# MECLabTUDA/Lifelong-nnUNet

Measured on AMD Instinct MI355X. Metric: 3D patches/sec (whole node) + mean Dice vs ref, 5-level 3D Generic_UNet training step, higher is better.
Workload: dtype f16 (fp32 accumulate, fp32 master weights); 1 GPU; BASELINE configs[1]: nnUNetTrainerSequential.run_iteration, 160x192x160 patches, batch 2/GPU, num_pool 5, base 32, 3 logits; global_batch=2, parallelism=dp1, distinct_resident_batches=2, deterministic_wgrad=False

## Files before the change

lifelong-nnunet_amd/csrc/igemm_common.h:

```cpp
#pragma once
#include "lnn_common.h"

struct TapTable {
    int ntaps;
    int taps_per_group;
    unsigned short pos_off[27];
    unsigned char slot[27];
};

struct ConvParams {
    const half_t* x;
    const half_t* x2;
    half_t* y2;
    int csplit = 0x7fffffff, msplit = 0x7fffffff;
    const half_t* wp;
    const float* bias;
    half_t* y;
    int ld_x, ld_y;
    int N, Di, Hi, Wi, Do, Ho, Wo;
    int C, M, Mpad, KCpad;
    int wtaps;
    int Ld, Lh, Lw;
    int tiles_z, tiles_y, tiles_x;
    int os, par_z, par_y, par_x;
// ... 8 lines not shown
    int gs_in[3] = {0, 0, 0}, gs_out[3] = {0, 0, 0};
    long gs_in_n = 0, gs_out_n = 0;
    unsigned gs_nrec_in = 0, gs_nrec_out = 0;
    int ksplit = 1;
    float* scratch = nullptr;
    unsigned long long* dbg;
    TapTable taps;
};


__host__ __device__ __forceinline__ long lnn_panel_off(int slot, int m, int kc, int wtaps, int KCpad) {
    return ((((long)(m >> 5) * (KCpad >> 4) + (kc >> 4)) * wtaps + slot) * 32 + (m & 31)) * 16 + (kc & 15);
}

int lnn_launch_conv_s1_tile(hipStream_t s, ConvParams& p, const char* name);
bool lnn_conv_s1_v9_supported(const ConvParams& p);
int lnn_conv_s1_v9_stats_slots(const ConvParams& p);
bool lnn_conv_s1_v9_red_supported(const ConvParams& p);
int lnn_launch_splitk_finalize(hipStream_t s, const ConvParams& p, const char* name);
int lnn_launch_in_small_fwd(hipStream_t s, const void* y, void* z, int ld_z, int N, long V, int C, float eps, const float* gamma,
                            const float* beta, float slope, float* mean, float* rstd);
int lnn_launch_in_small_bwd(hipStream_t s, void* y, const void* dz, int ld_dz, int N, long V, int C, const float* mean, const float* rstd,
                            const float* gamma, const float* beta, float slope, double* ws, float* dgamma, float* dbeta, float unscale);
int lnn_launch_in_stats_finalize(hipStream_t s, const float* pws, int nslots, int N, int C, long V, float eps, float* mean, float* rstd);
int lnn_launch_in_bwd_sums_raw(hipStream_t s, const float* pws, int nslots, int N, int C, const float* mean, const float* rstd,
                               double* ws, float* dgamma, float* dbeta, float unscale);
int lnn_launch_conv_s1_v9(hipStream_t s, ConvParams& p, const char* name);
int lnn_conv_k133_on_v9(hipStream_t s, const void* x, int ld_x, const void* wp, const float* bias, void* y, int ld_y, int N, int D, int H,
                        int W, int C, int M, int flip, const char* name);
bool lnn_conv_s1_mt_supported(const ConvParams& p);
double lnn_conv_s1_mt_efficiency(const ConvParams& p);
int lnn_conv_s1_mt_ksplit(const ConvParams& p, const float* ws, long ws_elems);
int lnn_launch_conv_s1_mt(hipStream_t s, ConvParams& p, float* ws, long ws_elems, const char* name);
int lnn_launch_up2_dgrad(hipStream_t s, ConvParams& p, const char* name);
int lnn_launch_up2_convT(hipStream_t s, ConvParams& p, const char* name);
int lnn_launch_down2_conv(hipStream_t s, ConvParams& p, const char* name);
int lnn_launch_down2_convT_dgrad(hipStream_t s, ConvParams& p, const char* name);
bool lnn_down2s_supported(const ConvParams& p);
int lnn_down2s_stats_slots(const ConvParams& p);
int lnn_launch_down2s(hipStream_t s, ConvParams& p, const char* name);
```

lifelong-nnunet_amd/csrc/igemm_conv.hip:

```cpp
#include "lnn_common.h"
#include "igemm_common.h"
#include "igemm_gen.h"
#include <cstdlib>

namespace {

typedef unsigned c1_uint4 __attribute__((ext_vector_type(4)));

template <bool STATS>
__global__ __launch_bounds__(256, 3) void conv_c1_fwd_kernel(const ConvParams p, int tiles_per_sample) {
    constexpr int TZ = 4, TY = 8, TX = 8, VT = TZ * TY * TX / 128, PZ = TZ + 2, PY = TY + 2, PX = TX + 2, P = PZ * PY * PX;
    constexpr int NL = (P + 255) / 256;
    __shared__ half_t xl[P];
    __shared__ float sred[STATS ? 4 * 2 * 32 : 1];
    const int tid = threadIdx.x, lane = tid & 63, wave = tid >> 6;
    const int n = blockIdx.y;
    const int m0 = blockIdx.z * 32;
    const long xbase_n = (long)n * p.Di * p.Hi * p.Wi;
    const int v = lane & 31, hk = lane >> 5;
    half8 a[2];
#pragma unroll
    for (int k16 = 0; k16 < 2; ++k16) a[k16] = *reinterpret_cast<const half8*>(p.wp + lnn_panel_off(0, m0 + v, k16 * 16 + hk * 8, 1, 32));
    int toff[2][8];
#pragma unroll
// ... 122 lines not shown
    if (v == 1) return true;
    static int min_planes = 0;
    if (!min_planes) { const char* e = getenv("LNN_CONV_V9_MIN_PLANES"); min_planes = e && atoi(e) > 0 ? atoi(e) : 16; }
    return p.Ld >= min_planes;
}

int g_force_down2 = -1;
bool use_down2s(const ConvParams& p) {
    if (!lnn_down2s_supported(p)) return false;
    if (g_force_down2 >= 0) return g_force_down2 == 1;
    static int v = -2;
    if (v == -2) {
        const char* e = getenv("LNN_DOWN2S");
        v = e ? (e[0] == '1' ? 1 : 0) : -1;
    }
    if (v == 0) return false;
    if (v == 1) return true;
    return p.Ld >= 16;
}

bool use_mt(const ConvParams& p) {
    if (!lnn_conv_s1_mt_supported(p)) return false;
    if (g_force_conv >= 0) return g_force_conv == 10;
    static int v = -2;
    if (v == -2) {
        const char* e = getenv("LNN_CONV_MT");
        v = e ? (e[0] == '1' ? 1 : 0) : -1;
    }
    if (v == 0) return false;
    if (v == 1) return true;
    return p.C >= 128;
}

}

static int g_gen_mode = -1;
extern "C" int lnn_debug_set_gen_mode(int mode) {
    LNN_REQUIRE(mode >= -1 && mode <= 1, "lnn_debug_set_gen_mode: %d is not one of -1, 0, 1", mode);
    g_gen_mode = mode;
    return LNN_OK;
}
bool lnn_gen_prefers(int op, long voxels) {
    if (g_gen_mode >= 0) return g_gen_mode == 1;
    if (g_force_conv >= 0) return false;
    static int off = -1;
    if (off < 0) { const char* e = getenv("LNN_GEN"); off = (e && e[0] == '0') ? 1 : 0; }
    if (off) return false;
    switch (op) {
        case LNN_GEN_OP_CONV_S1: return voxels > 512 && voxels <= 4096;
        case LNN_GEN_OP_CONV_S2: return voxels <= 4096;
        case LNN_GEN_OP_CONVT_DGRAD: return voxels <= 20000;
        default: return false;
    }
}

namespace {
int check_act(const void* ptr, int ld, int C, const char* what) {
    LNN_REQUIRE(ptr != nullptr, "%s: null pointer", what);
    LNN_REQUIRE(lnn_aligned16(ptr), "%s: pointer not 16-byte aligned", what);
    LNN_REQUIRE(C > 0 && C % 8 == 0, "%s: channel count %d must be a positive multiple of 8", what, C);
    LNN_REQUIRE(ld >= C && ld % 8 == 0, "%s: ld %d must be >= C (%d) and a multiple of 8", what, ld, C);
    return LNN_OK;
}

}

extern "C" int lnn_debug_force_down2_kernel(int which) {
    LNN_REQUIRE(which >= -1 && which <= 1, "lnn_debug_force_down2_kernel: %d is not one of -1, 0, 1", which);
    g_force_down2 = which;
    return LNN_OK;
}

extern "C" int lnn_debug_force_conv_kernel(int which) {
    LNN_REQUIRE(which == -1 || which == 5 || which == 9 || which == 10, "lnn_debug_force_conv_kernel: %d is not one of -1, 5, 9, 10", which);
    g_force_conv = which;
    return LNN_OK;
}

namespace {
int conv3d_fwd_impl(lnn_stream_t s_, const void* x, const void* x2, int c_a, int ld_x, const void* wp, const float* bias, void* y,
                    int ld_y, int N, int Di, int Hi, int Wi, int C, int K, int stride, float* stats_pws = nullptr,
                    int* stats_slots = nullptr, float* splitk_ws = nullptr, long splitk_elems = 0) {
    hipStream_t s = (hipStream_t)s_;
    LNN_REQUIRE(stride == 1 || stride == 2, "lnn_conv3d_fwd: stride %d unsupported", stride);
    LNN_REQUIRE(N > 0 && Di > 0 && Hi > 0 && Wi > 0, "lnn_conv3d_fwd: bad dims");
    LNN_REQUIRE(wp != nullptr && lnn_aligned16(wp), "lnn_conv3d_fwd: weight panel null/misaligned");
    LNN_REQUIRE(bias == nullptr || lnn_aligned16(bias), "lnn_conv3d_fwd: bias misaligned");
    if (int e = check_act(y, ld_y, K, "lnn_conv3d_fwd(y)")) return e;
    ConvParams p{};
    p.x = (const half_t*)x; p.wp = (const half_t*)wp; p.bias = bias; p.y = (half_t*)y;
    if (x2) { p.x2 = (const half_t*)x2; p.csplit = c_a; }
    p.ld_x = ld_x; p.ld_y = ld_y; p.N = N; p.Di = Di; p.Hi = Hi; p.Wi = Wi;
    p.Do = (Di - 1) / stride + 1; p.Ho = (Hi - 1) / stride + 1; p.Wo = (Wi - 1) / stride + 1;
    p.C = C; p.M = K; p.Mpad = lnn_round_up(K, 32); p.wtaps = C == 1 ? 1 : 27;
    p.Ld = p.Do; p.Lh = p.Ho; p.Lw = p.Wo; p.os = 1; p.pad_lo = 1; p.accumulate = 0;
    if (C == 1) {
        LNN_REQUIRE(stride == 1, "lnn_conv3d_fwd: C == 1 path supports stride 1 only");
        LNN_REQUIRE(x != nullptr, "lnn_conv3d_fwd: null x");
        p.KCpad = 32;
        p.tiles_z = lnn_cdiv(p.Ld, 4); p.tiles_y = lnn_cdiv(p.Lh, 8); p.tiles_x = lnn_cdiv(p.Lw, 8);
        const int tps = p.tiles_z * p.tiles_y * p.tiles_x;
        int nb = 768 / N;
        if (nb < 1) nb = 1;
        if (nb > tps) nb = tps;
        dim3 grid((unsigned)nb, (unsigned)N, (unsigned)lnn_cdiv(K, 32));
        if (stats_pws && ld_y == K) {
            p.stats_pws = stats_pws;
            p.stats_nblk = nb;
            hipLaunchKernelGGL((conv_c1_fwd_kernel<true>), grid, dim3(256), 0, s, p, tps);
            *stats_slots = nb;
        } else {
            hipLaunchKernelGGL((conv_c1_fwd_kernel<false>), grid, dim3(256), 0, s, p, tps);
        }
        LNN_CHECK_LAUNCH("lnn_conv3d_fwd(C=1)");
        return LNN_OK;
    }
    if (int e = check_act(x, ld_x, x2 ? c_a : C, "lnn_conv3d_fwd(x)")) return e;
    p.KCpad = lnn_round_up(C, 16);
    p.taps.ntaps = 27;
    if (stride == 1) {
        constexpr int PY = 10, PX = 10;
        for (int t = 0; t < 27; ++t) {
            p.taps.pos_off[t] = (unsigned short)(((t / 9) * PY + (t / 3) % 3) * PX + t % 3);
            p.taps.slot[t] = (unsigned char)t;
        }
        if (!use_v9(p) && use_mt(p)) return lnn_launch_conv_s1_mt(s, p, splitk_ws, splitk_elems, "lnn_conv3d_fwd(s1,mt)");
    }
    if (!x2 && lnn_gen_prefers(stride == 1 ? LNN_GEN_OP_CONV_S1 : LNN_GEN_OP_CONV_S2, (long)N * p.Do * p.Ho * p.Wo)) {
        const int k3[3] = {3, 3, 3}, st3[3] = {stride, stride, stride};
        return lnn_gen_conv3d_fwd(s, x, ld_x, wp, bias, y, ld_y, N, Di, Hi, Wi, C, K, k3, st3, splitk_ws, splitk_elems);
    }
    if (stride == 1) {
        p.dbg = g_dbg;
        if (stats_pws && use_v9(p) && ld_y == K && lnn_conv_s1_v9_stats_slots(p) <= 1024) {
            p.stats_pws = stats_pws;
            const int rc = lnn_launch_conv_s1_v9(s, p, "lnn_conv3d_fwd(s1,v9,stats)");
            *stats_slots = p.stats_nblk;
            return rc;
        }
        if (use_v9(p)) return lnn_launch_conv_s1_v9(s, p, "lnn_conv3d_fwd(s1,v9)");
        return lnn_launch_conv_s1_tile(s, p, "lnn_conv3d_fwd(s1,v5)");
    }
    if (use_down2s(p)) {
        if (stats_pws && ld_y == K && lnn_down2s_stats_slots(p) <= 1024) {
            p.stats_pws = stats_pws;
            const int rc = lnn_launch_down2s(s, p, "lnn_conv3d_fwd(s2,down2s,stats)");
            *stats_slots = p.stats_nblk;
            return rc;
        }
        return lnn_launch_down2s(s, p, "lnn_conv3d_fwd(s2,down2s)");
    }
    return lnn_launch_down2_conv(s, p, "lnn_conv3d_fwd(s2,down2)");
}

int check_cat(const void* b, int c_a, int C, int stride, const char* what) {
    LNN_REQUIRE(b != nullptr && lnn_aligned16(b), "%s: second tensor null/misaligned", what);
    LNN_REQUIRE(stride == 1, "%s: stride 1 only", what);
    LNN_REQUIRE(c_a > 0 && c_a < C && c_a % 32 == 0 && (C - c_a) % 8 == 0, "%s: split %d of %d channels must be a multiple of 32", what, c_a, C);
    return LNN_OK;
}
// ... 178 lines not shown
    hipStream_t s = (hipStream_t)s_;
    LNN_REQUIRE(wp != nullptr && lnn_aligned16(wp), "lnn_convT3d_k2s2_fwd: weight panel null/misaligned");
    if (int e = check_act(x, ld_x, C, "lnn_convT3d_k2s2_fwd(x)")) return e;
    if (int e = check_act(y, ld_y, K, "lnn_convT3d_k2s2_fwd(y)")) return e;
    if (lnn_gen_prefers(LNN_GEN_OP_CONVT_FWD, (long)N * D * H * W * 8)) {
        const int st3[3] = {2, 2, 2};
        return lnn_gen_convT3d_fwd(s, x, ld_x, wp, y, ld_y, N, D, H, W, C, K, st3, ws, ws_elems);
    }
    ConvParams p{};
    p.x = (const half_t*)x; p.wp = (const half_t*)wp; p.y = (half_t*)y; p.ld_x = ld_x; p.ld_y = ld_y;
    p.N = N; p.Di = D; p.Hi = H; p.Wi = W; p.Do = 2 * D; p.Ho = 2 * H; p.Wo = 2 * W;
    p.C = C; p.M = K; p.Mpad = lnn_round_up(K, 32); p.KCpad = lnn_round_up(C, 16); p.wtaps = 8;
    p.Ld = D; p.Lh = H; p.Lw = W; p.os = 2; p.pad_lo = 0;
    return lnn_launch_up2_convT(s, p, "lnn_convT3d_k2s2_fwd(up2)");
}
}

extern "C" int lnn_convT3d_k2s2_fwd(lnn_stream_t s, const void* x, int ld_x, const void* wp, void* y, int ld_y, int N,
                                    int D, int H, int W, int C, int K) {
    return convT3d_k2s2_fwd_impl(s, x, ld_x, wp, y, ld_y, N, D, H, W, C, K, nullptr, 0);
}
extern "C" int lnn_convT3d_k2s2_fwd_ws(lnn_stream_t s, const void* x, int ld_x, const void* wp, void* y, int ld_y, int N,
                                       int D, int H, int W, int C, int K, float* splitk_ws, long splitk_elems) {
    return convT3d_k2s2_fwd_impl(s, x, ld_x, wp, y, ld_y, N, D, H, W, C, K, splitk_ws, splitk_elems);
}

namespace {
int convT3d_k2s2_dgrad_impl(lnn_stream_t s_, const void* dy, int ld_dy, const void* wp, void* dx, int ld_dx, int N, int D, int H, int W,
                            int C, int K, int accumulate, float* ws, long ws_elems) {
    hipStream_t s = (hipStream_t)s_;
    LNN_REQUIRE(wp != nullptr && lnn_aligned16(wp), "lnn_convT3d_k2s2_dgrad: weight panel null/misaligned");
    if (int e = check_act(dy, ld_dy, K, "lnn_convT3d_k2s2_dgrad(dy)")) return e;
    if (int e = check_act(dx, ld_dx, C, "lnn_convT3d_k2s2_dgrad(dx)")) return e;
    if (lnn_gen_prefers(LNN_GEN_OP_CONVT_DGRAD, (long)N * D * H * W)) {
        const int st3[3] = {2, 2, 2};
        return lnn_gen_convT3d_dgrad(s, dy, ld_dy, wp, dx, ld_dx, N, D, H, W, C, K, st3, accumulate, ws, ws_elems);
    }
    ConvParams p{};
    p.x = (const half_t*)dy; p.wp = (const half_t*)wp; p.y = (half_t*)dx; p.ld_x = ld_dy; p.ld_y = ld_dx;
    p.N = N; p.Di = 2 * D; p.Hi = 2 * H; p.Wi = 2 * W; p.Do = D; p.Ho = H; p.Wo = W;
    p.C = K; p.M = C; p.Mpad = lnn_round_up(C, 32); p.KCpad = lnn_round_up(K, 16); p.wtaps = 8;
    p.Ld = D; p.Lh = H; p.Lw = W; p.os = 1; p.pad_lo = 0; p.accumulate = accumulate;
    if (use_down2s(p)) return lnn_launch_down2s(s, p, "lnn_convT3d_k2s2_dgrad(down2s)");
    return lnn_launch_down2_convT_dgrad(s, p, "lnn_convT3d_k2s2_dgrad(down2)");
}
}

extern "C" int lnn_convT3d_k2s2_dgrad(lnn_stream_t s, const void* dy, int ld_dy, const void* wp, void* dx, int ld_dx,
                                      int N, int D, int H, int W, int C, int K, int accumulate) {
    return convT3d_k2s2_dgrad_impl(s, dy, ld_dy, wp, dx, ld_dx, N, D, H, W, C, K, accumulate, nullptr, 0);
}
extern "C" int lnn_convT3d_k2s2_dgrad_ws(lnn_stream_t s, const void* dy, int ld_dy, const void* wp, void* dx, int ld_dx,
                                         int N, int D, int H, int W, int C, int K, int accumulate, float* splitk_ws, long splitk_elems) {
    return convT3d_k2s2_dgrad_impl(s, dy, ld_dy, wp, dx, ld_dx, N, D, H, W, C, K, accumulate, splitk_ws, splitk_elems);
}
```

lifelong-nnunet_amd/csrc/igemm_conv_mt.hip:

```cpp
#include "igemm_common.h"

namespace {

typedef unsigned uint4v __attribute__((ext_vector_type(4)));
typedef __attribute__((address_space(3))) void lds_void;

template <int N>
__device__ __forceinline__ void mt_wait_vm() {
    static_assert(N == 0 || N == 4 || N == 6 || N == 8 || N == 10 || N == 12, "extend the table");
    if constexpr (N == 0) asm volatile("s_waitcnt vmcnt(0)" ::: "memory");
    if constexpr (N == 4) asm volatile("s_waitcnt vmcnt(4)" ::: "memory");
    if constexpr (N == 6) asm volatile("s_waitcnt vmcnt(6)" ::: "memory");
    if constexpr (N == 8) asm volatile("s_waitcnt vmcnt(8)" ::: "memory");
    if constexpr (N == 10) asm volatile("s_waitcnt vmcnt(10)" ::: "memory");
    if constexpr (N == 12) asm volatile("s_waitcnt vmcnt(12)" ::: "memory");
}

__device__ __forceinline__ void mt_dma16(__amdgpu_buffer_rsrc_t rs, char* lds_wave_base, int voffset, int soffset) {
    __builtin_amdgcn_raw_ptr_buffer_load_lds(rs, (lds_void*)lds_wave_base, 16, voffset, soffset, 0, 0);
}

constexpr int MT_NW = 8;
constexpr int MT_NH = 4;
constexpr int MT_HALO = MT_NW * MT_NH * 1024;
constexpr int mt_lds(int AR) { return 2 * MT_HALO + MT_NW * AR * 2048; }
constexpr int MT_NIT = 7;

struct MTLaunch {
    int mblk;
    int zb, yb, xb;
    int TY, TX, PY, PX, P;
    int cpp;
    int nbands;
};

template <int WN, int MT_AR>
__global__ __launch_bounds__(512, 2) void igemm_conv_mt_kernel(const ConvParams p, const MTLaunch q) {
    static_assert(MT_AR >= 3 && MT_AR <= 7, "ring depth");
    extern __shared__ __attribute__((aligned(16))) char smem[];
    char* const aring = smem + 2 * MT_HALO;
    const int tid = threadIdx.x, lane = tid & 63;
    const int wave = __builtin_amdgcn_readfirstlane(tid >> 6);
    const int sub = wave >> 2, kq = wave & 3;
// ... 234 lines not shown
    }
    return lnn_cu_budget(num_cu);
}

bool mt_geometry(const ConvParams& p, int& WN, int& TY, int& TX, double& eff) {
    WN = 0; TY = 0; TX = 0; eff = 0.0;
    for (int nx = 1; nx <= 16; ++nx) {
        const int tx = lnn_cdiv(p.Lw, nx);
        if (nx > 1 && tx == lnn_cdiv(p.Lw, nx - 1)) continue;
        for (int wn = 5; wn >= 4; --wn) {
            int ty = (32 * wn) / tx;
            if (ty > p.Lh) ty = p.Lh;
            while (ty >= 1 && 4L * (ty + 2) * (tx + 2) > MT_NW * MT_NH * 32) --ty;
            if (ty < 1) continue;
            const double e = (double)p.Lh * p.Lw / ((double)lnn_cdiv(p.Lh, ty) * lnn_cdiv(p.Lw, tx) * 32 * wn);
            if (e > eff + 1e-9) { eff = e; WN = wn; TY = ty; TX = tx; }
        }
    }
    return WN != 0;
}

template <int WN, int AR>
int launch_mt(hipStream_t s, ConvParams& p, const MTLaunch& q, int grid, const char* name) {
    static bool attr_set = false;
    if (!attr_set) {
        (void)hipFuncSetAttribute(reinterpret_cast<const void*>(igemm_conv_mt_kernel<WN, AR>), hipFuncAttributeMaxDynamicSharedMemorySize, mt_lds(AR));
        attr_set = true;
    }
    hipLaunchKernelGGL((igemm_conv_mt_kernel<WN, AR>), dim3(grid), dim3(512), mt_lds(AR), s, p, q);
    LNN_CHECK_LAUNCH(name);
    return LNN_OK;
}

}

int lnn_launch_splitk_finalize(hipStream_t s, const ConvParams& p, const char* name) {
    const long nvox = (long)p.N * p.Do * p.Ho * p.Wo;
    const long total = nvox * (p.Mpad >> 2);
    const int blocks = (int)((total + 255) / 256 < 4096 ? (total + 255) / 256 : 4096);
    hipLaunchKernelGGL(splitk_finalize_kernel, dim3(blocks), dim3(256), 0, s, p, nvox);
    LNN_CHECK_LAUNCH(name);
    return LNN_OK;
}

bool lnn_conv_s1_mt_supported(const ConvParams& p) {
    if (p.os != 1 || p.pad_lo != 1 || p.taps.ntaps != 27 || p.wtaps != 27) return false;
    if (p.C % 16 != 0 || p.Mpad % 32 != 0 || p.M % 8 != 0) return false;
    if (p.ld_x % 8 != 0 || p.ld_y % 8 != 0) return false;
    if (p.csplit != 0x7fffffff && p.csplit % 16 != 0) return false;
    if (p.msplit != 0x7fffffff && p.msplit % 32 != 0) return false;
    if (p.Di != p.Do || p.Hi != p.Ho || p.Wi != p.Wo) return false;
    if ((double)p.Di * p.Hi * p.Wi * p.ld_x * 2.0 >= 2147483648.0) return false;
    if ((double)p.Mpad * p.KCpad * 27 * 2.0 >= 2147483648.0) return false;
    int wn, ty, tx; double eff;
    return mt_geometry(p, wn, ty, tx, eff);
}

double lnn_conv_s1_mt_efficiency(const ConvParams& p) {
    int wn, ty, tx; double eff;
    if (!lnn_conv_s1_mt_supported(p) || !mt_geometry(p, wn, ty, tx, eff)) return 0.0;
    return eff * p.Ld / (2.0 * lnn_cdiv(p.Ld, 2));
}

int lnn_conv_s1_mt_ksplit(const ConvParams& p, const float* ws, long ws_elems) {
    int wn, ty, tx; double eff;
    if (!mt_geometry(p, wn, ty, tx, eff)) return 1;
// ... 30 lines not shown
```

lifelong-nnunet_amd/csrc/lnn_debug.h:

```cpp
#ifndef LNN_DEBUG_H
#define LNN_DEBUG_H
#include "../../include/lnn_hip.h"
#ifdef __cplusplus
extern "C" {
#endif

int lnn_debug_tr16_probe(lnn_stream_t s, float* out256);

int lnn_debug_set_phase_buffer(void* dev_ptr_6x_u64);
int lnn_debug_force_conv_kernel(int which);
int lnn_debug_force_down2_kernel(int which);
int lnn_debug_set_v9_zseg(int segments);

int lnn_debug_set_k133_v9(int mode);
int lnn_debug_last_k133_on_v9(void);

int lnn_debug_set_gen_mode(int mode);

int lnn_debug_last_dgrad_reduce_fused(void);

int lnn_debug_set_cu_budget(int cus);

#ifdef __cplusplus
}
#endif
#endif
```

lifelong-nnunet_amd/engine.py:

```python
from __future__ import annotations

from dataclasses import dataclass, field
from typing import List, Optional

import os

import torch

from . import native as nat

LRELU_SLOPE = 1e-2
IN_EPS = 1e-5


class Act:

    def __init__(self, buf: torch.Tensor, off: int, C: int):
        self.buf, self.off, self.C = buf, off, C
        self.ld = buf.shape[-1]
        self.N = buf.shape[0]
        self.dims = tuple(buf.shape[1:4])
        self.V = self.dims[0] * self.dims[1] * self.dims[2]

    def data_ptr(self):
# ... 340 lines not shown
        self._pack_total, self._unpack_total = pk_total, up_total
        cmax = max(2 * f for f in feats)
        ws_doubles = max(nat.query("lnn_instnorm_ws_doubles", N, cmax), (nat.query("lnn_seg1x1_bwd_ws_floats", N, cmax) + 1) // 2,
                         nat.query("lnn_instnorm_lrelu_seg_bwd_ws_doubles", N, max(seg.cin for seg in self.segs)), 64)
        self.ws = torch.zeros(ws_doubles, dtype=torch.float64, device=dev)
        need = 1
        for blk in self.blocks:
            if blk.stride != 1 or blk.cin_k == 1:
                continue
            od = blk.in_dims
            vox = N * od[0] * od[1] * od[2]
            tiles = N * -(-od[0] // 8) * -(-od[1] // 8) * -(-od[2] // 8)
            for ch in (blk.cout, blk.cin):
                if tiles * -(-ch // 32) < 512:
                    need = max(need, 8 * vox * (-(-ch // 32) * 32))

        def gen_need(vox, ch, classes=1, always=False, limit=4096):
            if vox > limit and not always:
                return 1
            mp = -(-ch // 32) * 32
            waves = classes * -(-(vox // classes) // 64) * -(-mp // 64)
            ks = 1
            while waves * ks * 2 <= 2048 and ks < 64:
                ks *= 2
            return ks * vox * mp if ks > 1 else 1
        for blk in self.blocks:
            if blk.cin_k == 1:
                continue
            ncls = blk.strides[0] * blk.strides[1] * blk.strides[2]
            need = max(need, gen_need(N * blk.z.V, blk.cout, 1, not blk.iso))
            need = max(need, gen_need(N * blk.in_dims[0] * blk.in_dims[1] * blk.in_dims[2], blk.cin_k, ncls, not blk.iso))
        for up in self.ups:
            need = max(need, gen_need(N * up.y.V, up.cout, up.ntaps, not up.iso), gen_need(N * up.x.V, up.cin, 1, not up.iso, 20000))
        self.splitk_ws = torch.zeros(need, dtype=torch.float32, device=dev)
        self.packed_version = -1
        self.unused_heads: List[str] = []
        self._sides = {}
        self.overlap_wgrad = os.environ.get("LNN_NO_WGRAD_OVERLAP", "0") != "1"
        self.deterministic_wgrad = os.environ.get("LNN_DETERMINISTIC_WGRAD", "0") == "1"
        self._det_buf = None
        self.fuse_seg_fwd = os.environ.get("LNN_NO_FUSED_SEG", "0") != "1"
        self.numeric_conv_bias_grad = os.environ.get("LNN_NUMERIC_CONV_BIAS_GRAD", "0") == "1"
        self.fuse_in_stats = os.environ.get("LNN_NO_FUSED_IN_STATS", "0") != "1"
        self.fuse_seg_bwd = os.environ.get("LNN_NO_FUSED_SEG_BWD", "0") != "1"
        self.fuse_first_bwd = os.environ.get("LNN_NO_FUSED_FIRST_BWD", "0") != "1"
        self.fuse_in_bwd_reduce = os.environ.get("LNN_NO_FUSED_IN_BWD_REDUCE", "0") != "1"
        self.small_v = nat.query("lnn_instnorm_small_volume") if os.environ.get("LNN_IN_SMALL", "1") != "0" else 0
        self.probe = None
        self._watermark = {}
        for item in order:
            slots = [s for s in (getattr(item, a, None) for a in ("w", "b", "gamma", "beta")) if s is not None]
            self._watermark[id(item)] = max(s.offset + (s.numel + 3) // 4 * 4 for s in slots)

    def _probed(self, kind, item, fn):
        pr = self.probe
        if pr is None or (pr.get("layer") != item.prefix and pr.get("layer") != "*"):
            fn()
            return
        e0, e1 = torch.cuda.Event(enable_timing=True), torch.cuda.Event(enable_timing=True)
        e0.record()
        fn()
        e1.record()
        if pr.get("layer") == "*":
            pr.setdefault("all", []).append((item.prefix, kind, e0, e1))
        else:
            pr.setdefault(kind, []).append((e0, e1))
# ... 377 lines not shown
```

lifelong-nnunet_amd/native.py:

```python
from __future__ import annotations

import ctypes as C
import os

_HERE = os.path.dirname(os.path.abspath(__file__))
LIB_PATH = os.environ.get("LNN_LIB_PATH") or os.path.join(_HERE, "csrc", "liblnn_hip.so")

_p = C.c_void_p
_i = C.c_int
_l = C.c_long
_f = C.c_float
_sz = C.c_size_t

SIGNATURES = {
    "lnn_last_error": (C.c_char_p, []),
    "lnn_version": (_i, []),
    "lnn_device_info": (_i, [C.POINTER(_i), C.POINTER(_i), C.c_char_p, _i]),
    "lnn_pack_weights": (_i, [_p, _p, _p, _i, _i, _i, _l, _l, _l]),
    "lnn_packed_weight_elems": (_sz, [_i, _i, _i]),
    "lnn_conv3d_fwd": (_i, [_p, _p, _i, _p, _p, _p, _i, _i, _i, _i, _i, _i, _i, _i]),
    "lnn_conv3d_dgrad": (_i, [_p, _p, _i, _p, _p, _i, _i, _i, _i, _i, _i, _i, _i, _i]),
    "lnn_conv3d_wgrad": (_i, [_p, _p, _i, _p, _i, _p, _i, _i, _i, _i, _i, _i, _i]),
    "lnn_conv3d_fwd_cat": (_i, [_p, _p, _p, _i, _i, _p, _p, _p, _i, _i, _i, _i, _i, _i, _i]),
    "lnn_conv3d_fwd_in_stats": (_i, [_p, _p, _p, _i, _i, _p, _p, _p, _i, _i, _i, _i, _i, _i, _i, _f, _p, _p, _p, _p, _l]),
# ... 45 lines not shown
    "lnn_fisher_ema": (_i, [_p, _p, _p, _l, _f, _f]),
    "lnn_rw_update": (_i, [_p, _p, _p, _p, _p, _p, _l, _f, _f, _p, _f, _f, _i]),
    "lnn_target_ce_fwd": (_i, [_p, _p, _p, _i, _i, _i, _l, _f, _i, _f, _p, _p]),
    "lnn_target_ce_bwd": (_i, [_p, _p, _p, _i, _i, _i, _l, _f, _i, _f, _p, _f, _p, _p]),
    "lnn_softmax_accumulate": (_i, [_p, _p, _p, _p, _p] + [_i] * 11 + [_f, _i]),
    "lnn_softmax_finalize": (_i, [_p, _p, _p, _i, _l, _p]),
    "lnn_gradnorm_sumsq": (_i, [_p, _p, _l, _f, _p, _i]),
    "lnn_flat_reduce_ws_doubles": (_sz, []),
    "lnn_sgd_nesterov_step_clipped": (_i, [_p, _p, _p, _p, _l, _f, _f, _f, _f, _f, _p]),
    "lnn_sgd_nesterov_step": (_i, [_p, _p, _p, _p, _l, _f, _f, _f, _f, _i]),
    "lnn_cast_f32_to_h": (_i, [_p, _p, _p, _l]),
    "lnn_f32_conv3d_fwd": (_i, [_p, _p, _i, _p, _p, _p, _i, _i, _i, _i, _i, _i, _i, _i]),
    "lnn_f32_conv3d_dgrad": (_i, [_p, _p, _i, _p, _p, _i, _i, _i, _i, _i, _i, _i, _i, _i]),
    "lnn_f32_conv3d_wgrad": (_i, [_p, _p, _i, _p, _i, _p, _i, _i, _i, _i, _i, _i, _i]),
    "lnn_f32_convT3d_k2s2_fwd": (_i, [_p, _p, _i, _p, _p, _i, _i, _i, _i, _i, _i, _i]),
    "lnn_f32_convT3d_k2s2_dgrad": (_i, [_p, _p, _i, _p, _p, _i, _i, _i, _i, _i, _i, _i, _i]),
    "lnn_f32_convT3d_k2s2_wgrad": (_i, [_p, _p, _i, _p, _i, _p, _i, _i, _i, _i, _i, _i]),
    "lnn_f32_conv3d_fwd_g": (_i, [_p, _p, _i, _p, _p, _p, _i] + [_i] * 12),
    "lnn_f32_conv3d_dgrad_g": (_i, [_p, _p, _i, _p, _p, _i] + [_i] * 13),
    "lnn_f32_conv3d_wgrad_g": (_i, [_p, _p, _i, _p, _i, _p] + [_i] * 12),
    "lnn_f32_convT3d_fwd_g": (_i, [_p, _p, _i, _p, _p, _i] + [_i] * 9),
    "lnn_f32_convT3d_dgrad_g": (_i, [_p, _p, _i, _p, _p, _i] + [_i] * 10),
    "lnn_f32_convT3d_wgrad_g": (_i, [_p, _p, _i, _p, _i, _p] + [_i] * 9),
    "lnn_image_to_cl_h": (_i, [_p, _p, _p, _i, _i, _l, _i]),
    "lnn_f32_image_to_cl": (_i, [_p, _p, _p, _i, _i, _l, _i]),
    "lnn_f32_instnorm_lrelu_fwd": (_i, [_p, _p, _i, _p, _i, _i, _l, _i, _f, _p, _p, _p, _p, _f]),
    "lnn_f32_instnorm_lrelu_bwd": (_i, [_p, _p, _i, _p, _i, _i, _l, _i, _p, _p, _p, _p, _f, _p, _p, _p]),
    "lnn_f32_seg1x1_fwd": (_i, [_p, _p, _i, _p, _p, _i, _l, _i, _i]),
    "lnn_f32_seg1x1_bwd": (_i, [_p, _p, _i, _p, _p, _p, _i, _p, _i, _l, _i, _i, _i]),
    "lnn_debug_tr16_probe": (_i, [_p, _p]),
    "lnn_debug_set_phase_buffer": (_i, [_p]),
    "lnn_debug_force_conv_kernel": (_i, [_i]),
    "lnn_debug_force_down2_kernel": (_i, [_i]),
    "lnn_debug_set_v9_zseg": (_i, [_i]),
    "lnn_debug_set_k133_v9": (_i, [_i]),
    "lnn_debug_last_k133_on_v9": (_i, []),
    "lnn_debug_set_gen_mode": (_i, [_i]),
    "lnn_debug_last_dgrad_reduce_fused": (_i, []),
    "lnn_debug_set_cu_budget": (_i, [_i]),
    "lnn_conv3d_fwd_g": (_i, [_p, _p, _i, _p, _p, _p, _i] + [_i] * 12 + [_p, _l]),
    "lnn_conv3d_dgrad_g": (_i, [_p, _p, _i, _p, _p, _i] + [_i] * 13 + [_p, _l]),
    "lnn_conv3d_wgrad_g": (_i, [_p, _p, _i, _p, _i, _p] + [_i] * 12 + [_p, _l]),
    "lnn_convT3d_fwd_g": (_i, [_p, _p, _i, _p, _p, _i] + [_i] * 9 + [_p, _l]),
    "lnn_convT3d_dgrad_g": (_i, [_p, _p, _i, _p, _p, _i] + [_i] * 10 + [_p, _l]),
    "lnn_convT3d_wgrad_g": (_i, [_p, _p, _i, _p, _i, _p] + [_i] * 9 + [_p, _l]),
    "lnn_convT3d_k2s2_fwd_ws": (_i, [_p, _p, _i, _p, _p, _i, _i, _i, _i, _i, _i, _i, _p, _l]),
    "lnn_convT3d_k2s2_dgrad_ws": (_i, [_p, _p, _i, _p, _p, _i, _i, _i, _i, _i, _i, _i, _i, _p, _l]),
}

_lib = None


class NativeLibraryMissing(RuntimeError):
    pass


def lib():
    global _lib
    if _lib is None:
        if not os.path.exists(LIB_PATH):
            raise NativeLibraryMissing(
                f"{LIB_PATH} not found: build it with `python -c 'import __graft_entry__ as g; g.build()'` "
                f"(make -C lifelong-nnunet_amd/csrc).  There is no CPU / PyTorch fallback.")
        h = C.CDLL(LIB_PATH)
        for name, (res, args) in SIGNATURES.items():
            fn = getattr(h, name)
# ... 56 lines not shown
```

Baseline: 104.3 patches/s.

## Add stride-2 macro-tile implicit-GEMM kernel for downsampling conv and convT dgrad

Adds a new MFMA macro-tile kernel for stride-2 3x3x3 forward convolutions and 2x2x2 transposed-conv data gradients. It stages a phase-split halo band in LDS with double-buffered DMA and a ring of weight fragments, and splits taps across four waves followed by an LDS reduction. Optional split-K uses a scratch workspace, which is sized in the engine. It is chosen for iso layers with C>=128, more than 512 voxels and good tile efficiency, replacing the generic and down2 kernels there. This adds kernel complexity and LDS pressure and could pick a slower path on some shapes.

```diff
diff --git a/lifelong-nnunet_amd/csrc/igemm_common.h b/lifelong-nnunet_amd/csrc/igemm_common.h
--- a/lifelong-nnunet_amd/csrc/igemm_common.h
+++ b/lifelong-nnunet_amd/csrc/igemm_common.h
@@ -64,6 +64,10 @@
 double lnn_conv_s1_mt_efficiency(const ConvParams& p);
 int lnn_conv_s1_mt_ksplit(const ConvParams& p, const float* ws, long ws_elems);
 int lnn_launch_conv_s1_mt(hipStream_t s, ConvParams& p, float* ws, long ws_elems, const char* name);
+bool lnn_conv_s2_mt_supported(const ConvParams& p);
+double lnn_conv_s2_mt_efficiency(const ConvParams& p);
+long lnn_conv_s2_mt_scratch_elems(const ConvParams& p);
+int lnn_launch_conv_s2_mt(hipStream_t s, ConvParams& p, float* ws, long ws_elems, const char* name);
 int lnn_launch_up2_dgrad(hipStream_t s, ConvParams& p, const char* name);
 int lnn_launch_up2_convT(hipStream_t s, ConvParams& p, const char* name);
 int lnn_launch_down2_conv(hipStream_t s, ConvParams& p, const char* name);
diff --git a/lifelong-nnunet_amd/csrc/igemm_conv.hip b/lifelong-nnunet_amd/csrc/igemm_conv.hip
--- a/lifelong-nnunet_amd/csrc/igemm_conv.hip
+++ b/lifelong-nnunet_amd/csrc/igemm_conv.hip
@@ -178,6 +178,23 @@
     return p.C >= 128;
 }
 
+int g_last_s2_kernel = 0;
+int g_gen_mode_pinned();
+bool use_s2mt(const ConvParams& p, bool have_x2) {
+    if (have_x2 || !lnn_conv_s2_mt_supported(p)) return false;
+    if (g_force_down2 >= 0) return g_force_down2 == 2;
+    if (g_gen_mode_pinned() >= 0 || g_force_conv >= 0) return false;
+    static int v = -2;
+    if (v == -2) {
+        const char* e = getenv("LNN_CONV_S2MT");
+        v = e ? (e[0] == '1' ? 1 : 0) : -1;
+    }
+    if (v == 0) return false;
+    if (v == 1) return true;
+    const long vox = (long)p.N * p.Do * p.Ho * p.Wo;
+    return p.wtaps == 27 && p.C >= 128 && vox > 512 && lnn_conv_s2_mt_efficiency(p) >= 0.7;
+}
+
 }
 
 static int g_gen_mode = -1;
@@ -186,6 +203,7 @@
     g_gen_mode = mode;
     return LNN_OK;
 }
+namespace { int g_gen_mode_pinned() { return g_gen_mode; } }
 bool lnn_gen_prefers(int op, long voxels) {
     if (g_gen_mode >= 0) return g_gen_mode == 1;
     if (g_force_conv >= 0) return false;
@@ -212,9 +230,27 @@
 }
 
 extern "C" int lnn_debug_force_down2_kernel(int which) {
-    LNN_REQUIRE(which >= -1 && which <= 1, "lnn_debug_force_down2_kernel: %d is not one of -1, 0, 1", which);
+    LNN_REQUIRE(which >= -1 && which <= 2, "lnn_debug_force_down2_kernel: %d is not one of -1, 0, 1, 2", which);
     g_force_down2 = which;
     return LNN_OK;
+}
+extern "C" int lnn_debug_last_s2_kernel(void) { return g_last_s2_kernel; }
+
+extern "C" long lnn_conv_s2_mt_scratch_elems_q(int ext, int N, int D, int H, int W, int C, int K) {
+    ConvParams p{};
+    p.N = N; p.os = 1; p.ld_x = 8; p.ld_y = 8;
+    if (ext == 3) {
+        p.Di = D; p.Hi = H; p.Wi = W; p.Do = (D - 1) / 2 + 1; p.Ho = (H - 1) / 2 + 1; p.Wo = (W - 1) / 2 + 1;
+        p.C = C; p.M = K; p.wtaps = 27; p.pad_lo = 1; p.ld_x = lnn_round_up(C, 8);
+    } else if (ext == 2) {
+        p.Di = 2 * D; p.Hi = 2 * H; p.Wi = 2 * W; p.Do = D; p.Ho = H; p.Wo = W;
+        p.C = K; p.M = C; p.wtaps = 8; p.pad_lo = 0; p.ld_x = lnn_round_up(K, 8);
+    } else {
+        return 0;
+    }
+    p.Mpad = lnn_round_up(p.M, 32); p.KCpad = lnn_round_up(p.C, 16);
+    p.Ld = p.Do; p.Lh = p.Ho; p.Lw = p.Wo;
+    return lnn_conv_s2_mt_scratch_elems(p);
 }
 
 extern "C" int lnn_debug_force_conv_kernel(int which) {
@@ -272,6 +308,13 @@
         }
         if (!use_v9(p) && use_mt(p)) return lnn_launch_conv_s1_mt(s, p, splitk_ws, splitk_elems, "lnn_conv3d_fwd(s1,mt)");
     }
+    if (stride == 2) {
+        g_last_s2_kernel = 0;
+        if (use_s2mt(p, x2 != nullptr)) {
+            g_last_s2_kernel = 2;
+            return lnn_launch_conv_s2_mt(s, p, splitk_ws, splitk_elems, "lnn_conv3d_fwd(s2,mt)");
+        }
+    }
     if (!x2 && lnn_gen_prefers(stride == 1 ? LNN_GEN_OP_CONV_S1 : LNN_GEN_OP_CONV_S2, (long)N * p.Do * p.Ho * p.Wo)) {
         const int k3[3] = {3, 3, 3}, st3[3] = {stride, stride, stride};
         return lnn_gen_conv3d_fwd(s, x, ld_x, wp, bias, y, ld_y, N, Di, Hi, Wi, C, K, k3, st3, splitk_ws, splitk_elems);
@@ -516,15 +559,20 @@
     LNN_REQUIRE(wp != nullptr && lnn_aligned16(wp), "lnn_convT3d_k2s2_dgrad: weight panel null/misaligned");
     if (int e = check_act(dy, ld_dy, K, "lnn_convT3d_k2s2_dgrad(dy)")) return e;
     if (int e = check_act(dx, ld_dx, C, "lnn_convT3d_k2s2_dgrad(dx)")) return e;
-    if (lnn_gen_prefers(LNN_GEN_OP_CONVT_DGRAD, (long)N * D * H * W)) {
-        const int st3[3] = {2, 2, 2};
-        return lnn_gen_convT3d_dgrad(s, dy, ld_dy, wp, dx, ld_dx, N, D, H, W, C, K, st3, accumulate, ws, ws_elems);
-    }
     ConvParams p{};
     p.x = (const half_t*)dy; p.wp = (const half_t*)wp; p.y = (half_t*)dx; p.ld_x = ld_dy; p.ld_y = ld_dx;
     p.N = N; p.Di = 2 * D; p.Hi = 2 * H; p.Wi = 2 * W; p.Do = D; p.Ho = H; p.Wo = W;
     p.C = K; p.M = C; p.Mpad = lnn_round_up(C, 32); p.KCpad = lnn_round_up(K, 16); p.wtaps = 8;
     p.Ld = D; p.Lh = H; p.Lw = W; p.os = 1; p.pad_lo = 0; p.accumulate = accumulate;
+    g_last_s2_kernel = 0;
+    if (use_s2mt(p, false)) {
+        g_last_s2_kernel = 2;
+        return lnn_launch_conv_s2_mt(s, p, ws, ws_elems, "lnn_convT3d_k2s2_dgrad(s2,mt)");
+    }
+    if (lnn_gen_prefers(LNN_GEN_OP_CONVT_DGRAD, (long)N * D * H * W)) {
+        const int st3[3] = {2, 2, 2};
+        return lnn_gen_convT3d_dgrad(s, dy, ld_dy, wp, dx, ld_dx, N, D, H, W, C, K, st3, accumulate, ws, ws_elems);
+    }
     if (use_down2s(p)) return lnn_launch_down2s(s, p, "lnn_convT3d_k2s2_dgrad(down2s)");
     return lnn_launch_down2_convT_dgrad(s, p, "lnn_convT3d_k2s2_dgrad(down2)");
 }
diff --git a/lifelong-nnunet_amd/csrc/igemm_conv_mt.hip b/lifelong-nnunet_amd/csrc/igemm_conv_mt.hip
--- a/lifelong-nnunet_amd/csrc/igemm_conv_mt.hip
+++ b/lifelong-nnunet_amd/csrc/igemm_conv_mt.hip
@@ -7,8 +7,9 @@
 
 template <int N>
 __device__ __forceinline__ void mt_wait_vm() {
-    static_assert(N == 0 || N == 4 || N == 6 || N == 8 || N == 10 || N == 12, "extend the table");
+    static_assert(N == 0 || N == 2 || N == 4 || N == 6 || N == 8 || N == 10 || N == 12, "extend the table");
     if constexpr (N == 0) asm volatile("s_waitcnt vmcnt(0)" ::: "memory");
+    if constexpr (N == 2) asm volatile("s_waitcnt vmcnt(2)" ::: "memory");
     if constexpr (N == 4) asm volatile("s_waitcnt vmcnt(4)" ::: "memory");
     if constexpr (N == 6) asm volatile("s_waitcnt vmcnt(6)" ::: "memory");
     if constexpr (N == 8) asm volatile("s_waitcnt vmcnt(8)" ::: "memory");
@@ -309,6 +310,330 @@
     return LNN_OK;
 }
 
+constexpr int S2_NH = 6;
+constexpr int S2_HALO = MT_NW * S2_NH * 1024;
+constexpr int S2_AR = 4;
+constexpr int S2_LDS = 2 * S2_HALO + MT_NW * S2_AR * 2048;
+static_assert(S2_LDS <= 160 * 1024, "the stride-2 macro-tile kernel needs more LDS than a CU has");
+constexpr int S2_SUBP_MAX = MT_NW * S2_NH * 32 / 2;
+
+struct S2Launch {
+    int mblk, zb, yb, xb;
+    int TY, TX, PY, PX, SUBP;
+    int cpp, nbands;
+};
+
+template <int EXT, int WN>
+__global__ __launch_bounds__(512, 2) void igemm_conv_s2mt_kernel(const ConvParams p, const S2Launch q) {
+    constexpr int NDZ = EXT, IPT = EXT * EXT, WT = EXT * EXT * EXT, NIT = EXT == 3 ? 3 : 1, PAD = EXT == 3 ? 1 : 0, AR = S2_AR, NH = S2_NH;
+    static_assert(NIT == 1 || AR - 1 <= NIT, "the wait counts below assume at most one image DMA among the loads younger than a fragment");
+    extern __shared__ __attribute__((aligned(16))) char smem[];
+    char* const aring = smem + 2 * S2_HALO;
+    const int tid = threadIdx.x, lane = tid & 63;
+    const int wave = __builtin_amdgcn_readfirstlane(tid >> 6);
+    const int sub = wave >> 2, kq = wave & 3;
+    const int hk = lane >> 5, v = lane & 31;
+
+    int b = blockIdx.x;
+    if ((gridDim.x & 7) == 0) b = (b & 7) * (gridDim.x >> 3) + (b >> 3);
+    const int mb = b % q.mblk; b /= q.mblk;
+    const int band = b % q.nbands;
+    const int part = b / q.nbands;
+    const int xbi = band % q.xb, bzy = band / q.xb;
+    const int ybi = bzy % q.yb, zbi = (bzy / q.yb) % q.zb, n = bzy / (q.yb * q.zb);
+    const int z0 = zbi * 2, y0 = ybi * q.TY, x0 = xbi * q.TX;
+    const int m0 = mb * 64;
+    const int PX = q.PX, PYX = q.PY * q.PX;
+
+    int hvoff[NH], hsub[NH];
+#pragma unroll
+    for (int k = 0; k < NH; ++k) {
+        const int g0 = (wave * NH + k) * 32;
+        hsub[k] = g0 / q.SUBP;
+        const int pos = g0 + (lane >> 1);
+        const int pis = pos - hsub[k] * q.SUBP;
+        const int cls = pis / PYX, rem = pis - cls * PYX, jy = rem / PX, jx = rem - jy * PX;
+        const int cy = cls >> 1, cx = cls & 1;
+        const int iy = 2 * (y0 + jy - PAD) + cy, ix = 2 * (x0 + jx - PAD) + cx;
+        bool ok = hsub[k] < 2 && cls < 4 && (unsigned)iy < (unsigned)p.Hi && (unsigned)ix < (unsigned)p.Wi;
+        if (PAD && ((cy == 0 && jy == 0) || (cx == 0 && jx == 0))) ok = false;
+        const int half = (lane & 1) ^ ((pos >> 3) & 1);
+        hvoff[k] = ok ? ((iy * p.Wi + ix) * p.ld_x + half * 8) * 2 : (int)0x80000000;
+    }
+    const int plane_bytes = p.Hi * p.Wi * p.ld_x * 2;
+    const long sample_elems = (long)p.Di * p.Hi * p.Wi * p.ld_x;
+    const half_t* const xn = p.x + (long)n * sample_elems;
+    const int xbytes = (int)(sample_elems * 2);
+    const int c_begin = part * q.cpp, nvc = q.cpp * NDZ;
+    int hbuf = 0;
+    auto dma_halo = [&](int vc) {
+        const int dz = vc / q.cpp, ch = vc - dz * q.cpp;
+        const int cb = (c_begin + ch) * 32;
+#pragma unroll
+        for (int k = 0; k < NH; ++k) {
+            const int iz = 2 * (z0 + hsub[k]) + dz - PAD;
+            const bool zok = vc < nvc && hsub[k] < 2 && (unsigned)iz < (unsigned)p.Di;
+            __amdgpu_buffer_rsrc_t rs = __builtin_amdgcn_make_buffer_rsrc((void*)xn, 0, zok ? xbytes : 0, 0x00020000);
+            mt_dma16(rs, smem + hbuf + (wave * NH + k) * 1024, hvoff[k], zok ? cb + iz * plane_bytes : 0);
+        }
+        hbuf ^= S2_HALO;
+    };
+
+    const int avoff = ((((lane & 31) + 8 * kq) & 31) * 32 + hk * 16);
+    const int kc16 = p.KCpad >> 4;
+    const long rb_stride = (long)kc16 * WT * 512;
+    const bool rb1_live = m0 + 32 < p.Mpad;
+    bool taplive[NIT];
+    int toffb[NIT];
+#pragma unroll
+    for (int it = 0; it < NIT; ++it) {
+        const int t2 = kq * NIT + it;
+        taplive[it] = t2 < IPT;
+        const int dy = t2 / EXT, dx = t2 - dy * EXT;
+        int cls, oy, ox;
+        if (EXT == 3) { cls = (dy != 1) * 2 + (dx != 1); oy = dy != 0; ox = dx != 0; }
+        else { cls = dy * 2 + dx; oy = 0; ox = 0; }
+        toffb[it] = taplive[it] ? ((cls * q.PY + oy) * PX + ox) * 32 : 0;
+    }
+    const int wbytes = (int)((long)(p.Mpad >> 5) * rb_stride * 2);
+    const int wbase = (int)((long)(m0 >> 5) * rb_stride * 2), rb_bytes = (int)(rb_stride * 2);
+    int aslot = 0;
+    auto dma_a = [&](int it, int vc) {
+        const int dz = vc / q.cpp, ch = vc - dz * q.cpp;
+        const bool ok = vc < nvc && taplive[it];
+        const int so = ok ? wbase + ((c_begin + ch) * WT + dz * IPT + kq * NIT + it) * 1024 : 0;
+        const bool ok1 = ok && rb1_live;
+        __amdgpu_buffer_rsrc_t r0 = __builtin_amdgcn_make_buffer_rsrc((void*)p.wp, 0, ok ? wbytes : 0, 0x00020000);
+        __amdgpu_buffer_rsrc_t r1 = __builtin_amdgcn_make_buffer_rsrc((void*)p.wp, 0, ok1 ? wbytes : 0, 0x00020000);
+        char* dst = aring + wave * (AR * 2048) + aslot;
+        mt_dma16(r0, dst, avoff, so);
+        mt_dma16(r1, dst + 1024, avoff, ok1 ? so + rb_bytes : 0);
+        aslot = aslot + 2048 == AR * 2048 ? 0 : aslot + 2048;
+    };
+
+    const int nv = q.TY * q.TX;
+    int lb[WN];
+#pragma unroll
+    for (int ct = 0; ct < WN; ++ct) {
+        const int vv = ct * 32 + v;
+        const int vc = vv < nv ? vv : nv - 1;
+        const int yy = vc / q.TX, xx = vc - yy * q.TX;
+        lb[ct] = (sub * q.SUBP + yy * PX + xx) * 32 + hk * 16;
+    }
+
+    floatx16 acc[2][WN];
+#pragma unroll
+    for (int rb = 0; rb < 2; ++rb)
+#pragma unroll
+        for (int ct = 0; ct < WN; ++ct)
+#pragma unroll
+            for (int i = 0; i < 16; ++i) acc[rb][ct][i] = 0.f;
+
+    half8 fa[2][2], fb[WN];
+    int rslot = 0, rbuf = 0;
+    auto load_a = [&](int set) {
+        const char* ab = aring + wave * (AR * 2048) + rslot + lane * 16;
+        fa[set][0] = *reinterpret_cast<const half8*>(ab);
+        fa[set][1] = *reinterpret_cast<const half8*>(ab + 1024);
+        rslot = rslot + 2048 == AR * 2048 ? 0 : rslot + 2048;
+    };
+    auto load_b = [&](int it, int ct) {
+        const int bb = lb[ct] + rbuf + toffb[it];
+        fb[ct] = *reinterpret_cast<const half8*>(smem + (bb ^ ((bb >> 4) & 16)));
+    };
+
+    dma_halo(0);
+#pragma unroll
+    for (int i = 0; i < AR; ++i) dma_a(i % NIT, i / NIT);
+    mt_wait_vm<2 * (AR - 1)>();
+    __builtin_amdgcn_s_barrier();
+    dma_halo(1);
+
+#pragma unroll 1
+    for (int c = 0; c < nvc; ++c) {
+        load_a(0);
+#pragma unroll
+        for (int ct = 0; ct < WN; ++ct) load_b(0, ct);
+#pragma unroll
+        for (int it = 0; it < NIT; ++it) {
+            const int cur = it & 1, nxt = (it + 1) & 1;
+            if (it + 1 < NIT) {
+                mt_wait_vm<2 * (AR - 2) + NH>();
+                load_a(nxt);
+            }
+            __builtin_amdgcn_sched_barrier(0);
+#pragma unroll
+            for (int ct = 0; ct < WN; ++ct) {
+#pragma unroll
+                for (int rb = 0; rb < 2; ++rb)
+                    acc[rb][ct] = __builtin_amdgcn_mfma_f32_32x32x16_f16(fa[cur][rb], fb[ct], acc[rb][ct], 0, 0, 0);
+                if (it + 1 < NIT) load_b(it + 1, ct);
+                __builtin_amdgcn_sched_barrier(0);
+            }
+            dma_a((it + AR) % NIT, c + (it + AR) / NIT);
+        }
+        if (c + 1 < nvc) {
+            mt_wait_vm<2 * (AR - 1 < NIT ? AR - 1 : NIT)>();
+            __builtin_amdgcn_s_barrier();
+            rbuf ^= S2_HALO;
+            dma_halo(c + 2);
+        }
+    }
+    mt_wait_vm<0>();
+    __builtin_amdgcn_s_barrier();
+
+    const long nvox = (long)p.N * p.Do * p.Ho * p.Wo;
+    const long vbase = (long)n * p.Do * p.Ho * p.Wo;
+    int ooff[WN];
+#pragma unroll
+    for (int ct = 0; ct < WN; ++ct) {
+        const int vv = ct * 32 + v;
+        const int yy = vv / q.TX, xx = vv - yy * q.TX;
+        const int oz = z0 + sub, oy = y0 + yy, ox = x0 + xx;
+        ooff[ct] = (vv < nv && oz < p.Ld && oy < p.Lh && ox < p.Lw) ? ((oz * p.Ho + oy) * p.Wo + ox) : -1;
+    }
+#pragma unroll
+    for (int rb = 0; rb < 2; ++rb) {
+        if (rb) __builtin_amdgcn_s_barrier();
+#pragma unroll
+        for (int a = 1; a < 4; ++a) {
+            const int Q = (a + kq) & 3;
+            char* dst = smem + (((sub * 4 + Q) * 3 + (3 - a)) * WN) * 1024 + lane * 16;
+#pragma unroll
+            for (int ct = 0; ct < WN; ++ct) {
+                const floatx4 w = {acc[rb][ct][4 * a], acc[rb][ct][4 * a + 1], acc[rb][ct][4 * a + 2], acc[rb][ct][4 * a + 3]};
+                *reinterpret_cast<floatx4*>(dst + ct * 1024) = w;
+            }
+        }
+        asm volatile("s_waitcnt lgkmcnt(0)" ::: "memory");
+        __builtin_amdgcn_s_barrier();
+        const char* src = smem + (((sub * 4 + kq) * 3) * WN) * 1024 + lane * 16;
+        const int m = m0 + rb * 32 + 8 * kq + 4 * hk;
+        const bool m_ok = m < p.M;
+        floatx4 bv = {0.f, 0.f, 0.f, 0.f};
+        if (p.bias && p.ksplit == 1 && m_ok) bv = *reinterpret_cast<const floatx4*>(p.bias + m);
+#pragma unroll
+        for (int ct = 0; ct < WN; ++ct) {
+            floatx4 r = {acc[rb][ct][0], acc[rb][ct][1], acc[rb][ct][2], acc[rb][ct][3]};
+#pragma unroll
+            for (int s = 0; s < 3; ++s) r += *reinterpret_cast<const floatx4*>(src + (s * WN + ct) * 1024);
+            if (ooff[ct] < 0 || !m_ok) continue;
+            const long vox = vbase + ooff[ct];
+            if (p.ksplit > 1) {
+                *reinterpret_cast<floatx4*>(p.scratch + ((long)part * nvox + vox) * p.Mpad + m) = r;
+                continue;
+            }
+            r += bv;
+            half4* dst = reinterpret_cast<half4*>(p.y + vox * p.ld_y + m);
+            if (p.accumulate) {
+                const half4 old = *dst;
+                r[0] += (float)old[0]; r[1] += (float)old[1]; r[2] += (float)old[2]; r[3] += (float)old[3];
+            }
+            const half4 o = {(half_t)r[0], (half_t)r[1], (half_t)r[2], (half_t)r[3]};
+            *dst = o;
+        }
+    }
+}
+
+bool s2mt_geometry(const ConvParams& p, int ext, int& WN, int& TY, int& TX, double& eff) {
+    const int pad = ext == 3 ? 1 : 0;
+    WN = 0; TY = 0; TX = 0; eff = 0.0;
+    for (int nx = 1; nx <= 16; ++nx) {
+        const int tx = lnn_cdiv(p.Lw, nx);
+        if (nx > 1 && tx == lnn_cdiv(p.Lw, nx - 1)) continue;
+        for (int wn = 5; wn >= 4; --wn) {
+            int ty = (32 * wn) / tx;
+            if (ty > p.Lh) ty = p.Lh;
+            while (ty >= 1 && 4L * (ty + pad) * (tx + pad) > S2_SUBP_MAX) --ty;
+            if (ty < 1) continue;
+            const double e = (double)p.Lh * p.Lw / ((double)lnn_cdiv(p.Lh, ty) * lnn_cdiv(p.Lw, tx) * 32 * wn);
+            if (e > eff + 1e-9) { eff = e; WN = wn; TY = ty; TX = tx; }
+        }
+    }
+    return WN != 0;
+}
+
+int s2mt_ext(const ConvParams& p) { return p.wtaps == 27 ? 3 : p.wtaps == 8 ? 2 : 0; }
+
+template <int EXT, int WN>
+int launch_s2mt(hipStream_t s, ConvParams& p, const S2Launch& q, int grid, const char* name) {
+    static bool attr_set[64] = {};
+    int dev = 0;
+    LNN_REQUIRE(hipGetDevice(&dev) == hipSuccess && dev >= 0 && dev < 64, "%s: no current device", name);
+    if (!attr_set[dev]) {
+        const hipError_t e = hipFuncSetAttribute(reinterpret_cast<const void*>(igemm_conv_s2mt_kernel<EXT, WN>),
+                                                 hipFuncAttributeMaxDynamicSharedMemorySize, S2_LDS);
+        LNN_REQUIRE(e == hipSuccess, "%s: device %d refuses %d bytes of dynamic LDS (%s)", name, dev, S2_LDS, hipGetErrorString(e));
+        attr_set[dev] = true;
+    }
+    hipLaunchKernelGGL((igemm_conv_s2mt_kernel<EXT, WN>), dim3(grid), dim3(512), S2_LDS, s, p, q);
+    LNN_CHECK_LAUNCH(name);
+    return LNN_OK;
+}
+
+}
+
+bool lnn_conv_s2_mt_supported(const ConvParams& p) {
+    const int ext = s2mt_ext(p);
+    if (!ext || p.os != 1 || p.pad_lo != (ext == 3 ? 1 : 0) || p.x2 || p.y2) return false;
+    if (p.C % 16 != 0 || p.KCpad != p.C || p.Mpad % 32 != 0 || p.M % 8 != 0) return false;
+    if (p.ld_x % 8 != 0 || p.ld_y % 8 != 0) return false;
+    if (p.Ld != p.Do || p.Lh != p.Ho || p.Lw != p.Wo) return false;
+    if (ext == 3 && (p.Di < 2 || p.Hi < 2 || p.Wi < 2 || p.Do != (p.Di - 1) / 2 + 1 || p.Ho != (p.Hi - 1) / 2 + 1 || p.Wo != (p.Wi - 1) / 2 + 1)) return false;
+    if (ext == 2 && (p.Di != 2 * p.Do || p.Hi != 2 * p.Ho || p.Wi != 2 * p.Wo)) return false;
+    if ((double)p.Di * p.Hi * p.Wi * p.ld_x * 2.0 >= 2147483648.0) return false;
+    if ((double)p.Mpad * p.KCpad * ext * ext * ext * 2.0 >= 2147483648.0) return false;
+    int wn, ty, tx; double eff;
+    return s2mt_geometry(p, ext, wn, ty, tx, eff);
+}
+
+double lnn_conv_s2_mt_efficiency(const ConvParams& p) {
+    int wn, ty, tx; double eff;
+    if (!lnn_conv_s2_mt_supported(p) || !s2mt_geometry(p, s2mt_ext(p), wn, ty, tx, eff)) return 0.0;
+    return eff * p.Ld / (2.0 * lnn_cdiv(p.Ld, 2));
+}
+
+int lnn_conv_s2_mt_ksplit(const ConvParams& p, const float* ws, long ws_elems, bool unlimited) {
+    int wn, ty, tx; double eff;
+    if (!s2mt_geometry(p, s2mt_ext(p), wn, ty, tx, eff)) return 1;
+    const long items = (long)lnn_cdiv(p.Mpad, 64) * p.N * lnn_cdiv(p.Ld, 2) * lnn_cdiv(p.Lh, ty) * lnn_cdiv(p.Lw, tx);
+    const int nchunks = p.C / 16;
+    const long nvox = (long)p.N * p.Do * p.Ho * p.Wo;
+    const int cus = mt_num_cu();
+    if (!ws && !unlimited) return 1;
+    int best = 1;
+    for (int k = 2; k <= 16; ++k)
+        if (nchunks % k == 0 && nchunks / k >= 2 && items * k <= cus + cus / 16 && (unlimited || ws_elems >= (long)k * nvox * p.Mpad)) best = k;
+    return items * 2 <= cus ? best : 1;
+}
+
+long lnn_conv_s2_mt_scratch_elems(const ConvParams& p) {
+    if (!lnn_conv_s2_mt_supported(p)) return 0;
+    const int ks = lnn_conv_s2_mt_ksplit(p, nullptr, 0, true);
+    return ks > 1 ? (long)ks * p.N * p.Do * p.Ho * p.Wo * p.Mpad : 0;
+}
+
+int lnn_launch_conv_s2_mt(hipStream_t s, ConvParams& p, float* ws, long ws_elems, const char* name) {
+    LNN_REQUIRE(lnn_conv_s2_mt_supported(p), "%s: shape not supported by the stride-2 macro-tile kernel", name);
+    const int ext = s2mt_ext(p), pad = ext == 3 ? 1 : 0;
+    int WN, TY, TX; double eff;
+    s2mt_geometry(p, ext, WN, TY, TX, eff);
+    S2Launch q;
+    q.mblk = lnn_cdiv(p.Mpad, 64);
+    q.zb = lnn_cdiv(p.Ld, 2); q.yb = lnn_cdiv(p.Lh, TY); q.xb = lnn_cdiv(p.Lw, TX);
+    q.TY = TY; q.TX = TX; q.PY = TY + pad; q.PX = TX + pad; q.SUBP = lnn_round_up(4 * q.PY * q.PX, 32);
+    LNN_REQUIRE(q.SUBP <= S2_SUBP_MAX, "%s: band image of %d positions", name, q.SUBP);
+    q.nbands = p.N * q.zb * q.yb * q.xb;
+    const int ks = lnn_conv_s2_mt_ksplit(p, ws, ws_elems, false);
+    p.ksplit = ks;
+    p.scratch = ks > 1 ? ws : nullptr;
+    q.cpp = (p.C / 16) / ks;
+    const int grid = q.mblk * q.nbands * ks;
+    int rc;
+    if (ext == 3) rc = WN == 5 ? launch_s2mt<3, 5>(s, p, q, grid, name) : launch_s2mt<3, 4>(s, p, q, grid, name);
+    else rc = WN == 5 ? launch_s2mt<2, 5>(s, p, q, grid, name) : launch_s2mt<2, 4>(s, p, q, grid, name);
+    if (rc != LNN_OK || ks == 1) return rc;
+    return lnn_launch_splitk_finalize(s, p, name);
 }
 
 int lnn_launch_splitk_finalize(hipStream_t s, const ConvParams& p, const char* name) {
diff --git a/lifelong-nnunet_amd/csrc/lnn_debug.h b/lifelong-nnunet_amd/csrc/lnn_debug.h
--- a/lifelong-nnunet_amd/csrc/lnn_debug.h
+++ b/lifelong-nnunet_amd/csrc/lnn_debug.h
@@ -10,6 +10,8 @@
 int lnn_debug_set_phase_buffer(void* dev_ptr_6x_u64);
 int lnn_debug_force_conv_kernel(int which);
 int lnn_debug_force_down2_kernel(int which);
+int lnn_debug_last_s2_kernel(void);
+long lnn_conv_s2_mt_scratch_elems_q(int ext, int N, int D, int H, int W, int C, int K);
 int lnn_debug_set_v9_zseg(int segments);
 
 int lnn_debug_set_k133_v9(int mode);
diff --git a/lifelong-nnunet_amd/engine.py b/lifelong-nnunet_amd/engine.py
--- a/lifelong-nnunet_amd/engine.py
+++ b/lifelong-nnunet_amd/engine.py
@@ -396,6 +396,12 @@
             need = max(need, gen_need(N * blk.in_dims[0] * blk.in_dims[1] * blk.in_dims[2], blk.cin_k, ncls, not blk.iso))
         for up in self.ups:
             need = max(need, gen_need(N * up.y.V, up.cout, up.ntaps, not up.iso), gen_need(N * up.x.V, up.cin, 1, not up.iso, 20000))
+        for blk in self.blocks:
+            if blk.iso and blk.stride == 2 and blk.cin_k != 1:
+                need = max(need, nat.query("lnn_conv_s2_mt_scratch_elems_q", 3, N, *blk.in_dims, blk.cin_k, blk.cout))
+        for up in self.ups:
+            if up.iso:
+                need = max(need, nat.query("lnn_conv_s2_mt_scratch_elems_q", 2, N, *up.x.dims, up.cin, up.cout))
         self.splitk_ws = torch.zeros(need, dtype=torch.float32, device=dev)
         self.packed_version = -1
         self.unused_heads: List[str] = []
diff --git a/lifelong-nnunet_amd/native.py b/lifelong-nnunet_amd/native.py
--- a/lifelong-nnunet_amd/native.py
+++ b/lifelong-nnunet_amd/native.py
@@ -101,6 +101,8 @@
     "lnn_debug_set_phase_buffer": (_i, [_p]),
     "lnn_debug_force_conv_kernel": (_i, [_i]),
     "lnn_debug_force_down2_kernel": (_i, [_i]),
+    "lnn_debug_last_s2_kernel": (_i, []),
+    "lnn_conv_s2_mt_scratch_elems_q": (_l, [_i, _i, _i, _i, _i, _i, _i]),
     "lnn_debug_set_v9_zseg": (_i, [_i]),
     "lnn_debug_set_k133_v9": (_i, [_i]),
     "lnn_debug_last_k133_on_v9": (_i, []),
```

Result: no change. 104.8 patches/s (median of 6 runs) (+0.5%).
